# Shahriar1638/Hybrid-Language-Music-Clustering-VAE

Hardware: AMD Instinct MI355X
Metric: clips/sec mel+VAE train step, 128-mel x 128-frame, bs=256, 1/2/4/8 MI355X (higher is better)
Workload: dtype bf16; 1 GPU; Convolutional_VAE audio-only (BASELINE config[1]): PCM[256,65024] -> HIP mel-dB 128x128 -> z-score -> VAE fwd+bwd+Adam; per_gpu_batch=256, global_batch=256, mel=128x128, params=13304961, parallelism=dp1, world_size=1, launch=single process, pcm_batches=5 distinct batches in rotation (333 MB), execution=eager launches

## Files before the change

hybrid-language-music-clustering-vae_amd/csrc/gemm.hpp:

```cpp
#pragma once
#include "common.hpp"

namespace hlmc {

constexpr int kKCH = 8;
template <typename T>
constexpr int gemm_bk() { return kKCH * Vec16<T>::N; }

__device__ __forceinline__ int xcd_logical_block(int lin, int total) {
    const int xcd = lin & 7, idx = lin >> 3;
    const int q = total >> 3, r = total & 7;
    return (xcd < r ? xcd * (q + 1) : r * (q + 1) + (xcd - r) * q) + idx;
}

static __device__ __attribute__((aligned(16))) uint4 g_zero16 = {0u, 0u, 0u, 0u};
template <typename T> __device__ __attribute__((aligned(16))) uint4 g_one16 = {sizeof(T) == 2 ? 0x3F80u : 0x3F800000u, 0u, 0u, 0u};


template <typename T>
struct DenseLoader {
    const T* p;
    int ld, M, Kd;
    bool vec;
    struct Row {
// ... 29 lines not shown
    int Hi, Wi, C, Ho, Wo, M;
    int cshift;
    FastDiv dWo, dHo;
    struct Row {
        int64_t base;
        int flags;
    };
    struct Ctx {
        int64_t off;
        int reject;
    };
    __device__ void set_phase(int) {}
    __device__ int K() const { return 9 * C; }
    __device__ Row prep(int m) const {
        if (m >= M) return Row{0, 1 | 8};
        const int t = (int)dWo.div((uint32_t)m), ow = m - t * Wo;
        const int b = (int)dHo.div((uint32_t)t), oh = t - b * Ho;
        return Row{(((int64_t)b * Hi + 2 * oh - 1) * Wi + 2 * ow - 1) * C, 8 | (oh == 0 ? 2 : 0) | (ow == 0 ? 4 : 0)};
    }
    __device__ Ctx ctx(int k) const {
        const int tap = cshift >= 0 ? (k >> cshift) : k / C;
        const int ci = k - tap * C;
        const int kh = tap / 3, kw = tap - kh * 3;
        return Ctx{((int64_t)kh * Wi + kw) * C + ci, 1 | (kh == 0 ? 2 : 0) | (kw == 0 ? 4 : 0) | (tap >= 9 ? 8 : 0)};
    }
    __host__ __device__ bool vec_ok() const { return true; }
    __device__ uint4 load(const Row& rw, const Ctx& cx) const { return *reinterpret_cast<const uint4*>(addr(rw, cx)); }
    __device__ const void* addr(const Row& rw, const Ctx& cx) const {
        if (rw.flags & cx.reject) return &g_zero16;
        return x + rw.base + cx.off;
    }
};

__device__ __forceinline__ int sp_ntaps(int par) { return par ? 2 : 1; }
__device__ __forceinline__ int sp_kidx(int par, int t) { return par ? (t ? 2 : 0) : 1; }
__device__ __forceinline__ int sp_delta(int par, int t) { return (par && t == 0) ? 1 : 0; }

template <typename T>
struct SubpixelLoader {
    const T* x;
    int Hi, Wi, C, M;
    int cshift;
    int py, px, ntx, Kd;
    FastDiv dWi, dHi;
    struct Row {
        int64_t base;
        int flags;
    };
    struct Ctx {
        int64_t off;
        int reject;
    };
    __device__ void set_phase(int p) {
        py = p >> 1; px = p & 1;
        ntx = sp_ntaps(px);
        Kd = sp_ntaps(py) * ntx * C;
    }
    __device__ int K() const { return Kd; }
    __device__ Row prep(int m) const {
        if (m >= M) return Row{0, 1 | 8};
        const int t = (int)dWi.div((uint32_t)m), c = m - t * Wi;
        const int b = (int)dHi.div((uint32_t)t), r = t - b * Hi;
        return Row{(((int64_t)b * Hi + r) * Wi + c) * C, 8 | (r == Hi - 1 ? 2 : 0) | (c == Wi - 1 ? 4 : 0)};
    }
    __device__ Ctx ctx(int k) const {
        const int tt = cshift >= 0 ? (k >> cshift) : k / C;
        const int ci = k - tt * C;
        const int ty = ntx == 2 ? (tt >> 1) : tt, tx = ntx == 2 ? (tt & 1) : 0;
        const int dr = sp_delta(py, ty), dc = sp_delta(px, tx);
        return Ctx{((int64_t)dr * Wi + dc) * C + ci, 1 | (dr ? 2 : 0) | (dc ? 4 : 0) | (k >= Kd ? 8 : 0)};
    }
    __host__ __device__ bool vec_ok() const { return true; }
    __device__ uint4 load(const Row& rw, const Ctx& cx) const { return *reinterpret_cast<const uint4*>(addr(rw, cx)); }
    __device__ const void* addr(const Row& rw, const Ctx& cx) const {
        if (rw.flags & cx.reject) return &g_zero16;
        return x + rw.base + cx.off;
    }
};

template <typename T>
struct SubpixelWeight {
    const T* w;
    int C, N;
    int cshift;
    int py, px, ntx, Kd;
    struct Row {
        const T* r;
    };
    struct Ctx {
        int off;
    };
    __device__ void set_phase(int p) {
        py = p >> 1; px = p & 1;
        ntx = sp_ntaps(px);
        Kd = sp_ntaps(py) * ntx * C;
    }
    __device__ int K() const { return Kd; }
    __device__ Row prep(int n) const { return Row{n < N ? w + (int64_t)n * 9 * C : nullptr}; }
    __device__ Ctx ctx(int k) const {
        if (k >= Kd) return Ctx{-1};
        const int tt = cshift >= 0 ? (k >> cshift) : k / C;
        const int ci = k - tt * C;
        const int ty = ntx == 2 ? (tt >> 1) : tt, tx = ntx == 2 ? (tt & 1) : 0;
        return Ctx{(sp_kidx(py, ty) * 3 + sp_kidx(px, tx)) * C + ci};
    }
    __host__ __device__ bool vec_ok() const { return true; }
    __device__ uint4 load(const Row& rw, const Ctx& cx) const { return *reinterpret_cast<const uint4*>(addr(rw, cx)); }
    __device__ const void* addr(const Row& rw, const Ctx& cx) const {
        if (!rw.r || cx.off < 0) return &g_zero16;
        return rw.r + cx.off;
    }
};

template <typename OutT>
__device__ __forceinline__ void store4_round(OutT* p, float (&v)[4]) {
    if constexpr (sizeof(OutT) == 4) {
        *reinterpret_cast<float4*>(p) = make_float4(v[0], v[1], v[2], v[3]);
    } else {
        unsigned h[4];
#pragma unroll
        for (int k = 0; k < 4; ++k) {
            bf16 t = __float2bfloat16(v[k]);
            h[k] = *reinterpret_cast<unsigned short*>(&t);
            v[k] = __uint_as_float(h[k] << 16);
        }
        *reinterpret_cast<uint2*>(p) = make_uint2(h[0] | (h[1] << 16), h[2] | (h[3] << 16));
    }
}

template <typename OutT>
struct StoreRM {
    static constexpr int kStatMode = 0;
    static constexpr bool kDirectTn = true;
    OutT* out;
    const float* bias;
    int ld, act, accumulate;
    struct Row {
        OutT* r;
    };
    struct Quad {
        int64_t off;
    };
    __device__ void set_split(int) {}
    __device__ float colbias(int n) const { return bias ? bias[n] : 0.f; }
    __device__ Quad quad(int m) const { return Quad{(int64_t)m * ld}; }
    __device__ int64_t row_off(const Quad& q, int r) const { return q.off + (int64_t)r * ld; }
    __device__ float put(int64_t ro, int n, float v) const {
        if (act == 1) v = v > 0.f ? v : 0.f;
        OutT* o = out + ro + n;
        if (accumulate) v += to_f32<OutT>(*o);
        const OutT t = from_f32<OutT>(v);
        *o = t;
        return to_f32<OutT>(t);
    }
    __device__ void put4(int64_t ro, int n, float (&v)[4]) const {
        OutT* o = out + ro + n;
#pragma unroll
        for (int k = 0; k < 4; ++k) {
            if (act == 1) v[k] = v[k] > 0.f ? v[k] : 0.f;
            if (accumulate) v[k] += to_f32<OutT>(o[k]);
        }
        store4_round<OutT>(o, v);
    }
    __device__ float put_na(int64_t ro, int n, float v) const {
        if (act == 1) v = v > 0.f ? v : 0.f;
        const OutT t = from_f32<OutT>(v);
        out[ro + n] = t;
        return to_f32<OutT>(t);
    }
    __device__ float stored(int n, float v) const {
        if (bias) v += bias[n];
        if (act == 1) v = v > 0.f ? v : 0.f;
        return to_f32<OutT>(from_f32<OutT>(v));
    }
    __device__ void set_phase(int) {}
    __device__ Row row(int m) const { return Row{out + (int64_t)m * ld}; }
// ... 98 lines not shown
    }
    __device__ float stored(int n, float v) const {
        if (this->bias) v += this->bias[n];
        return to_f32<OutT>(from_f32<OutT>(v));
    }
    __device__ Row row(int m) const { return Row{m, fx.flat_row(m)}; }
    __device__ void store(const Row& rw, int n, float v) const {
        if (this->bias) v += this->bias[n];
        put_at(rw.m, rw.base, n, v);
    }
};

template <typename OutT>
struct StoreSubpixel {
    static constexpr int kStatMode = 0;
    OutT* out;
    const float* bias;
    int Hi, Wi, N;
    int py, px;
    FastDiv dWi, dHi;
    struct Row {
        OutT* r;
    };
    struct Quad {
        int64_t off;
        int m;
    };
    __device__ int64_t pix_off(int m) const {
        const int t = (int)dWi.div((uint32_t)m), c = m - t * Wi;
        const int b = (int)dHi.div((uint32_t)t), r = t - b * Hi;
        return (((int64_t)b * 2 * Hi + 2 * r + py) * (2 * Wi) + 2 * c + px) * N;
    }
    __device__ void set_split(int) {}
    __device__ float colbias(int n) const { return bias ? bias[n] : 0.f; }
    __device__ Quad quad(int m) const { return Quad{pix_off(m), m}; }
    __device__ int64_t row_off(const Quad& q, int r) const {
        return (Wi & 3) == 0 ? q.off + (int64_t)2 * r * N : pix_off(q.m + r);
    }
    __device__ float put(int64_t ro, int n, float v) const {
        const OutT t = from_f32<OutT>(v);
        out[ro + n] = t;
        return to_f32<OutT>(t);
    }
    __device__ void put4(int64_t ro, int n, float (&v)[4]) const { store4_round<OutT>(out + ro + n, v); }
    __device__ float put_na(int64_t ro, int n, float v) const { return put(ro, n, v); }
    __device__ float stored(int n, float v) const {
        if (bias) v += bias[n];
        return to_f32<OutT>(from_f32<OutT>(v));
    }
    __device__ void set_phase(int p) { py = p >> 1; px = p & 1; }
    __device__ Row row(int m) const {
        const int c = m % Wi, t = m / Wi;
        const int r = t % Hi, b = t / Hi;
        const int64_t pix = ((int64_t)b * 2 * Hi + 2 * r + py) * (2 * Wi) + 2 * c + px;
        return Row{out + pix * N};
    }
    __device__ void store(const Row& rw, int n, float v) const {
        if (bias) v += bias[n];
        rw.r[n] = from_f32<OutT>(v);
    }
};

template <class Base>
struct WithStats : Base {
    static constexpr int kStatMode = 1;
    XAcc acc;
};
template <class EP>
inline WithStats<EP> with_stats(const EP& ep, const XAcc& acc) {
    WithStats<EP> eps;
    static_cast<EP&>(eps) = ep;
    eps.acc = acc;
    return eps;
}

struct StorePartial {
    static constexpr int kStatMode = 0;
    float* ws;
    int M, N, S;
    int phase, split;
    struct Row {
        float* r;
    };
    __device__ void set_phase(int p) { phase = p; }
    __device__ Row row(int m) const { return Row{ws + (((int64_t)phase * S + split) * M + m) * N}; }
    __device__ void store(const Row& rw, int n, float v) const { rw.r[n] = v; }
    struct Quad {
        int64_t off;
    };
    __device__ void set_split(int z) { split = z; }
    __device__ float colbias(int) const { return 0.f; }
    __device__ Quad quad(int m) const { return Quad{(((int64_t)phase * S + split) * M + m) * N}; }
    __device__ int64_t row_off(const Quad& q, int r) const { return q.off + (int64_t)r * N; }
    __device__ float put(int64_t ro, int n, float v) const {
        ws[ro + n] = v;
        return v;
    }
    __device__ void put4(int64_t ro, int n, float (&v)[4]) const {
        *reinterpret_cast<float4*>(ws + ro + n) = make_float4(v[0], v[1], v[2], v[3]);
    }
};

template <int TM, int TN, class EP>
__device__ __forceinline__ void epilogue_tile(const EP& ep, const f32x4_t (&acc)[TM][TN], int mb, int nb, int lane,
                                              int M, int N, double (&cs)[TN], double (&cq)[TN]) {
    float bias[TN];
    int ncol[TN];
#pragma unroll
    for (int j = 0; j < TN; ++j) {
        ncol[j] = nb + j * 16 + (lane & 15);
        bias[j] = ncol[j] < N ? ep.colbias(ncol[j]) : 0.f;
        cs[j] = 0.0;
        cq[j] = 0.0;
    }
#pragma unroll
    for (int i = 0; i < TM; ++i) {
        const int m = mb + i * 16 + (lane >> 4) * 4;
        if (m >= M) continue;
        const typename EP::Quad q = ep.quad(m);
#pragma unroll
        for (int r = 0; r < 4; ++r) {
            if (m + r >= M) continue;
            const int64_t ro = ep.row_off(q, r);
#pragma unroll
            for (int j = 0; j < TN; ++j) {
// ... 74 lines not shown
                    sred[(wmi * 2 + 1) * BN + wn0 + j * 16 + 4 * (lane >> 4) + k] = cq[j * 4 + k];
                }
        }
    } else {
#pragma unroll
        for (int j = 0; j < TN; ++j) {
            double a = cs[j], q = cq[j];
            a += __shfl_xor(a, 16, 64);
            q += __shfl_xor(q, 16, 64);
            a += __shfl_xor(a, 32, 64);
            q += __shfl_xor(q, 32, 64);
            if (lane < 16) {
                sred[(wmi * 2 + 0) * BN + wn0 + j * 16 + lane] = a;
                sred[(wmi * 2 + 1) * BN + wn0 + j * 16 + lane] = q;
            }
        }
    }
}
template <bool TR>
__device__ __forceinline__ f32x4_t mfma_bf16(const bf16x8_t& a, const bf16x8_t& b, const f32x4_t& c) {
    if constexpr (TR) return __builtin_amdgcn_mfma_f32_16x16x32_bf16(b, a, c, 0, 0, 0);
    else return __builtin_amdgcn_mfma_f32_16x16x32_bf16(a, b, c, 0, 0, 0);
}
template <bool TR>
__device__ __forceinline__ f32x4_t mfma_f32(float a, float b, const f32x4_t& c) {
    if constexpr (TR) return __builtin_amdgcn_mfma_f32_16x16x4f32(b, a, c, 0, 0, 0);
    else return __builtin_amdgcn_mfma_f32_16x16x4f32(a, b, c, 0, 0, 0);
}

#define NT_BLOCK_COORDS()                                                                                  \
    const int gx_ = (int)gridDim.x, gy_ = (int)gridDim.y;                                                  \
    const int lin_ = (int)blockIdx.x + gx_ * ((int)blockIdx.y + gy_ * (int)blockIdx.z);                     \
    const int lg_ = remap ? xcd_logical_block(lin_, gx_ * gy_ * (int)gridDim.z) : 0;                       \
    const int phase = remap ? lg_ % gy_ : (int)blockIdx.y;                                                 \
    const int tile_ = remap ? (lg_ / gy_) % gx_ : (int)blockIdx.x;                                         \
    const int bz = remap ? lg_ / (gx_ * gy_) : (int)blockIdx.z;                                            \
    const int m0 = (tile_ / tiles_n) * BM, n0 = (tile_ % tiles_n) * BN;                                     \
    const int tile_m_ = tile_ / tiles_n

template <int KCH>
__device__ __forceinline__ int nt_lds_chunk(int row, int c) {
    if constexpr (KCH == 8) return c ^ (row & 7);
    else return c ^ ((0x78 >> (2 * ((row >> 2) & 3))) & 3);
}

template <typename T, int BM, int BN, int WM, int WN, int KCH, class AL, class BL, class EP, bool TR = false>
__global__ __launch_bounds__(256) void gemm_nt_kernel(AL al, BL bl, EP ep, int M, int N, int ksplit_len, int remap,
                                                      int ploop) {
    constexpr int V = Vec16<T>::N;
    constexpr int BK = KCH * V;
    constexpr int WAVES_N = BN / WN;
    static_assert((BM / WM) * WAVES_N == 4, "4 waves per block");
    constexpr int TM = WM / 16, TN = WN / 16;
    constexpr int ACH = BM * KCH, BCH = BN * KCH;
    constexpr int AR = (ACH + 255) / 256, BR = (BCH + 255) / 256;
    __shared__ __attribute__((aligned(16))) T As[2][BM * BK];
    __shared__ __attribute__((aligned(16))) T Bs[2][BN * BK];

    const int tid = threadIdx.x, lane = tid & 63, wave = tid >> 6;
    const int wm0 = (wave / WAVES_N) * WM, wn0 = (wave % WAVES_N) * WN;
    const int tiles_n = (N + BN - 1) / BN;
    NT_BLOCK_COORDS();
    typename AL::Row arow[AR];
    typename BL::Row brow[BR];
#pragma unroll
    for (int i = 0; i < AR; ++i) arow[i] = al.prep(m0 + ((tid + i * 256) / KCH));
#pragma unroll
    for (int i = 0; i < BR; ++i) brow[i] = bl.prep(n0 + ((tid + i * 256) / KCH));
    const int ph0 = ploop > 1 ? 0 : phase, ph1 = ploop > 1 ? ploop : phase + 1;
// ... 137 lines not shown
#pragma unroll
            for (int w = 0; w < WAVES_M; ++w) {
                a += sred[w][0][c];
                q += sred[w][1][c];
            }
            xacc_add_shard(ep.acc, shard, n, a);
            xacc_add_shard(ep.acc, shard, N + n, q);
        }
    }
    if (ph + 1 < ph1) __syncthreads();
    }
}

template <int N>
__device__ __forceinline__ void wait_vmcnt() {
    static_assert(N >= 0 && N < 64, "vmcnt range");
    asm volatile("s_waitcnt vmcnt(%0)" ::"n"(N) : "memory");
}
template <int GPW, int NS>
__device__ __forceinline__ void wait_stage(int ahead) {
    if constexpr (NS >= 4) {
        if (ahead >= 2) { wait_vmcnt<2 * GPW>(); return; }
    }
    if constexpr (NS >= 3) {
        if (ahead >= 1) { wait_vmcnt<GPW>(); return; }
    }
    wait_vmcnt<0>();
}
__device__ __forceinline__ void glds16(const void* g, void* l) {
    __builtin_amdgcn_global_load_lds((const __attribute__((address_space(1))) void*)g,
                                     (__attribute__((address_space(3))) void*)l, 16, 0, 0);
}

template <typename T, int BM, int BN, int WM, int WN, int NS, class AL, class BL, class EP, bool TR = false, int WPE = 1>
__global__ __launch_bounds__(256) __attribute__((amdgpu_waves_per_eu(WPE))) void gemm_nt_glds_kernel(
    AL al, BL bl, EP ep, int M, int N, int ksplit_len, int remap) {
    constexpr int V = Vec16<T>::N;
    constexpr int BK = 8 * V;
    constexpr int ASZ = BM * 128, BSZ = BN * 128, STG = ASZ + BSZ;
    constexpr int AI = BM / 8, BI = BN / 8;
    static_assert(AI % 4 == 0 && BI >= 4 && BI % 4 == 0, "tile rows per stage must split over 4 waves");
    constexpr int AIW = AI / 4, BIW = BI / 4, GPW = AIW + BIW;
    constexpr int WAVES_N = BN / WN;
    static_assert((BM / WM) * WAVES_N == 4, "4 waves per block");
    constexpr int TM = WM / 16, TN = WN / 16;
    __shared__ __attribute__((aligned(1024))) char smem[NS * STG];

    const int tid = threadIdx.x, lane = tid & 63, wave = tid >> 6;
    const int wm0 = (wave / WAVES_N) * WM, wn0 = (wave % WAVES_N) * WN;
    const int tiles_n = (N + BN - 1) / BN;
    NT_BLOCK_COORDS();
    al.set_phase(phase); bl.set_phase(phase); ep.set_phase(phase); ep.set_split(bz);
    const int K = al.K();
    const int kb = bz * ksplit_len;
    const int ke = min(K, kb + ksplit_len);
    const int nsteps = kb < ke ? (ke - kb + BK - 1) / BK : 0;

    f32x4_t acc[TM][TN];
#pragma unroll
    for (int i = 0; i < TM; ++i)
#pragma unroll
        for (int j = 0; j < TN; ++j) acc[i][j] = f32x4_t{0.f, 0.f, 0.f, 0.f};

    const int lrow = lane >> 3;
    const int lchunk = (lane & 7) ^ (lrow & 7);
    typename AL::Row arow[AIW];
    typename BL::Row brow[BIW];
#pragma unroll
    for (int i = 0; i < AIW; ++i) arow[i] = al.prep(m0 + (wave * AIW + i) * 8 + lrow);
#pragma unroll
    for (int i = 0; i < BIW; ++i) brow[i] = bl.prep(n0 + (wave * BIW + i) * 8 + lrow);
    auto issue = [&](int slot, int k0) {
        char* sb = smem + slot * STG;
        const int k = k0 + lchunk * V;
        const typename AL::Ctx ax = al.ctx(k);
        const typename BL::Ctx bx = bl.ctx(k);
#pragma unroll
        for (int i = 0; i < AIW; ++i) glds16(al.addr(arow[i], ax), sb + (wave * AIW + i) * 1024);
#pragma unroll
        for (int i = 0; i < BIW; ++i) glds16(bl.addr(brow[i], bx), sb + ASZ + (wave * BIW + i) * 1024);
    };

#pragma unroll
    for (int p = 0; p < NS - 1; ++p)
// ... 18 lines not shown
                for (int j = 0; j < TN; ++j) {
                    const int row = wn0 + j * 16 + (lane & 15);
                    bfr[j] = *reinterpret_cast<const bf16x8_t*>(sbb + row * 128 + ((c ^ (row & 7)) << 4));
                }
#pragma unroll
                for (int i = 0; i < TM; ++i)
#pragma unroll
                    for (int j = 0; j < TN; ++j)
                        acc[i][j] = mfma_bf16<TR>(af[i], bfr[j], acc[i][j]);
            }
        } else {
#pragma unroll
            for (int s = 0; s < BK / 4; ++s) {
                float af[TM], bfr[TN];
                const int q = lane >> 4;
#pragma unroll
                for (int i = 0; i < TM; ++i) {
                    const int row = wm0 + i * 16 + (lane & 15);
                    af[i] = *reinterpret_cast<const float*>(sa + row * 128 + ((s ^ (row & 7)) << 4) + q * 4);
                }
#pragma unroll
                for (int j = 0; j < TN; ++j) {
                    const int row = wn0 + j * 16 + (lane & 15);
                    bfr[j] = *reinterpret_cast<const float*>(sbb + row * 128 + ((s ^ (row & 7)) << 4) + q * 4);
                }
#pragma unroll
                for (int i = 0; i < TM; ++i)
#pragma unroll
                    for (int j = 0; j < TN; ++j)
                        acc[i][j] = mfma_f32<TR>(af[i], bfr[j], acc[i][j]);
            }
        }
    }
    double cs[TR ? TN * 4 : TN], cq[TR ? TN * 4 : TN];
    if constexpr (TR)
        epilogue_tile_t<TM, TN, EP, sizeof(T) == 2>(ep, acc, m0 + wm0, n0 + wn0, lane, M, N,
                                *reinterpret_cast<double(*)[TN][4]>(cs), *reinterpret_cast<double(*)[TN][4]>(cq));
    else
        epilogue_tile<TM, TN>(ep, acc, m0 + wm0, n0 + wn0, lane, M, N, cs, cq);
    if constexpr (EP::kStatMode != 0) {
        constexpr int WAVES_M = BM / WM;
        static_assert(WAVES_M * 2 * BN * 8 <= NS * STG, "stats scratch fits the staging ring");
        __syncthreads();
        double* sred = reinterpret_cast<double*>(smem);
        const int wmi = wave / WAVES_N;
        stats_to_lds<TR, TN, BN>(cs, cq, sred, wmi, wn0, lane);
        __syncthreads();
        const int shard = (int)((blockIdx.x + gridDim.x * blockIdx.y) % (unsigned)ep.acc.shards);
        for (int c = tid; c < BN; c += 256) {
            const int n = n0 + c;
            if (n >= N) continue;
            double a = 0.0, q = 0.0;
#pragma unroll
            for (int w = 0; w < WAVES_M; ++w) {
                a += sred[(w * 2 + 0) * BN + c];
                q += sred[(w * 2 + 1) * BN + c];
            }
            xacc_add_shard(ep.acc, shard, n, a);
            xacc_add_shard(ep.acc, shard, N + n, q);
        }
    }
}

struct StorePartialZ : StorePartial {
    __device__ void set_split(int z) { split = z; }
};

template <int VW>
using slab_t = std::conditional_t<VW == 4, float4, float>;
__device__ __forceinline__ void slab_add(float& a, float b) { a += b; }
__device__ __forceinline__ void slab_add(float4& a, const float4& b) { a.x += b.x; a.y += b.y; a.z += b.z; a.w += b.w; }
__device__ __forceinline__ float slab_at(float v, int) { return v; }
__device__ __forceinline__ float slab_at(const float4& v, int i) { return i == 0 ? v.x : i == 1 ? v.y : i == 2 ? v.z : v.w; }
template <int VW, int G, class I>
__device__ __forceinline__ slab_t<VW> slab_sum(const float* __restrict__ p, I st, int S, int g) {
    using V = slab_t<VW>;
    auto ld = [&](int k) { return *reinterpret_cast<const V*>(p + k * st); };
    V acc{};
    int k = g;
    for (; k + 3 * G < S; k += 4 * G) {
        const V a0 = ld(k), a1 = ld(k + G), a2 = ld(k + 2 * G), a3 = ld(k + 3 * G);
        slab_add(acc, a0); slab_add(acc, a1); slab_add(acc, a2); slab_add(acc, a3);
    }
    for (; k < S; k += G) slab_add(acc, ld(k));
    return acc;
}
template <class EP>
__device__ __forceinline__ void slab_store(const EP& ep, int ph, int m, int n, float v) {
    EP e = ep;
    e.set_phase(ph);
    e.store(e.row(m), n, v);
}
template <class EP>
__device__ __forceinline__ void slab_store(const EP& ep, int ph, int m, int n, const float4& v) {
    EP e = ep;
    e.set_phase(ph);
    const auto rw = e.row(m);
    e.store(rw, n, v.x);
    e.store(rw, n + 1, v.y);
    e.store(rw, n + 2, v.z);
    e.store(rw, n + 3, v.w);
}

template <int VW, class EP>
__global__ __launch_bounds__(256) void splitk_reduce_kernel(const float* __restrict__ ws, EP ep, int M, int N, int S,
                                                            int phases, FastDiv dN, FastDiv dM) {
    if constexpr (VW == 4) {
        const uint32_t e = (blockIdx.x * 256u + threadIdx.x) * 4u;
        if (e >= (uint32_t)phases * (uint32_t)M * (uint32_t)N) return;
        const uint32_t t = dN.div(e), n = e - t * (uint32_t)N;
        const uint32_t ph = dM.div(t), m = t - ph * (uint32_t)M;
        const uint32_t st = (uint32_t)M * (uint32_t)N;
        const float* p = ws + ((ph * (uint32_t)S) * (uint32_t)M + m) * (uint32_t)N + n;
        slab_store(ep, (int)ph, (int)m, (int)n, slab_sum<4, 1>(p, st, S, 0));
    } else {
        const int64_t total = (int64_t)phases * M * N, st = (int64_t)M * N;
        for (int64_t i = (int64_t)blockIdx.x * blockDim.x + threadIdx.x; i < total; i += (int64_t)gridDim.x * blockDim.x) {
            const int n = (int)(i % N);
            const int64_t t = i / N;
            const int m = (int)(t % M), ph = (int)(t / M);
            slab_store(ep, ph, m, n, slab_sum<1, 1>(ws + ((int64_t)ph * S * M + m) * N + n, st, S, 0));
        }
    }
}

template <class EP, int RU>
__global__ __launch_bounds__(256) void splitk_reduce_stats_kernel(const float* ws, EP ep, int M, int N, int S,
                                                                  int phases, XAcc acc) {
    __shared__ double red[2][256];
    const int tid = threadIdx.x, c = tid & 63, g = tid >> 6;
    const int ntc = N >> 6;
    const int tr = (int)(blockIdx.x / (unsigned)ntc);
    const int col = ((int)blockIdx.x - tr * ntc) * 64 + c;
    const int rows = phases * M;
    const unsigned st = (unsigned)M * (unsigned)N;
    const int r0 = tr * 4 * RU + g;
    unsigned off[RU];
    float s[RU];
#pragma unroll
    for (int u = 0; u < RU; ++u) {
        const int r = min(r0 + 4 * u, rows - 1);
        const int ph = r / M, m = r - ph * M;
        off[u] = ((unsigned)(ph * S) * (unsigned)M + (unsigned)m) * (unsigned)N + (unsigned)col;
        s[u] = 0.f;
    }
    int k = 0;
    for (; k + 2 <= S; k += 2) {
        float x0[RU], x1[RU];
#pragma unroll
        for (int u = 0; u < RU; ++u) {
            x0[u] = ws[off[u] + (unsigned)k * st];
            x1[u] = ws[off[u] + (unsigned)(k + 1) * st];
        }
#pragma unroll
        for (int u = 0; u < RU; ++u) {
            s[u] += x0[u];
            s[u] += x1[u];
        }
    }
    if (k < S)
#pragma unroll
        for (int u = 0; u < RU; ++u) s[u] += ws[off[u] + (unsigned)k * st];
    double a = 0.0, q = 0.0;
#pragma unroll
    for (int u = 0; u < RU; ++u) {
        const int r = r0 + 4 * u;
        if (r >= rows) break;
        const int ph = r / M, m = r - ph * M;
        EP e = ep;
        e.set_phase(ph);
        e.store(e.row(m), col, s[u]);
        const float v = e.stored(col, s[u]);
        a += v;
        q += (double)v * v;
    }
    red[0][tid] = a;
    red[1][tid] = q;
    __syncthreads();
    if (tid < 64) {
#pragma unroll
        for (int j = 1; j < 4; ++j) {
            a += red[0][j * 64 + tid];
            q += red[1][j * 64 + tid];
        }
        xacc_add(acc, col, a);
        xacc_add(acc, N + col, q);
    }
}

template <class L>
struct KRowStepped {
    struct Pre {
        typename L::Col cl;
        int j;
    };
// ... 414 lines not shown
```

hybrid-language-music-clustering-vae_amd/csrc/gemm_ops.hip:

```cpp
#include "gemm.hpp"
#include "halo.hpp"
#include "ops.hpp"

#include <algorithm>
#include <type_traits>
#include <cstdlib>

namespace hlmc {
namespace {

constexpr int kNtTargetBlocks = 512;
constexpr int kTnTargetBlocks = 192;
constexpr int kTnLongK = 131072;
constexpr int kTnKch8Min = 1024;
constexpr int kXcdRemapKinds = probe::kWgradS2 | probe::kLinearWgrad;

struct Plan {
    int S, ksl;
};
template <int BM_, int BN_, int WM_, int WN_>
struct Tile {
    static constexpr int BM = BM_, BN = BN_, WM = WM_, WN = WN_;
};
struct GemmPlan {
    int tiles;
    Plan pl;
    size_t slab_bytes;
};
inline Plan plan_nt(int tiles, int Kmax, int BK) {
    constexpr int target = kNtTargetBlocks;
    int S = 1;
    if (tiles < target / 2) {
        S = cdiv(target, tiles);
        S = std::min(S, std::max(1, Kmax / (2 * BK)));
    }
    int ksl = cdiv(cdiv(Kmax, S), BK) * BK;
    S = cdiv(Kmax, ksl);
    return {S, ksl};
}
inline Plan plan_tn(int tiles, int K, int BK) {
    const int target = K >= kTnLongK ? 2 * kTnTargetBlocks : kTnTargetBlocks;
    int S = cdiv(target, tiles);
    S = std::max(1, std::min(S, K / (4 * BK)));
    int ksl = cdiv(cdiv(K, S), BK) * BK;
    S = cdiv(K, ksl);
    return {S, ksl};
}

constexpr int kGldsSplitMax = 512;
inline int nt_pipe_select(int ksl, int S, int blocks) {
    if (S > 1 && blocks <= kGldsSplitMax) return 2;
    return ksl >= 1024 ? 2 : 0;
}

inline int xcd_remap_for_site() { return (kXcdRemapKinds & probe::g_site.kind) ? 1 : 0; }

constexpr int kPloopTiles = 1024;
inline bool use_ploop(int phases, int tmn, int pipe) { return phases >= 2 && pipe == 0 && tmn >= kPloopTiles; }

template <typename T, class TL, bool TR, class AL, class BL, class E>
void nt_kernel_launch_tr(hipStream_t s, dim3 grid, const AL& al, const BL& bl, const E& ep, int M, int N, int ksl,
                         bool long_k, int pipe) {
    constexpr int BM = TL::BM, BN = TL::BN, WM = TL::WM, WN = TL::WN;
    const int rm = xcd_remap_for_site();
    const int ploop = use_ploop((int)grid.y, (int)grid.x, pipe) ? (int)grid.y : 1;
    if (ploop > 1) grid.y = 1;
    HLMC_PROBE_BEGIN(s);
    if (pipe == 2)
        gemm_nt_glds_kernel<T, BM, BN, WM, WN, 2, AL, BL, E, TR, 2><<<grid, 256, 0, s>>>(al, bl, ep, M, N, ksl, rm);
    else if (long_k)
        gemm_nt_kernel<T, BM, BN, WM, WN, 8, AL, BL, E, TR><<<grid, 256, 0, s>>>(al, bl, ep, M, N, ksl, rm, ploop);
    else
        gemm_nt_kernel<T, BM, BN, WM, WN, 4, AL, BL, E, TR><<<grid, 256, 0, s>>>(al, bl, ep, M, N, ksl, rm, ploop);
    HLMC_PROBE_END(s);
}

template <typename T, class TL>
GemmPlan nt_plan(int M, int N, int Kmax, int phases) {
    const int tmn = cdiv(M, TL::BM) * cdiv(N, TL::BN);
    const Plan pl = plan_nt(tmn * phases, Kmax, gemm_bk<T>());
    return {tmn, pl, (size_t)phases * pl.S * M * N * sizeof(float)};
}
inline bool nt_long_k(int Kmax) { return Kmax >= 1024; }

template <typename T, class TL, bool TR, class AL, class BL>
int nt_partials(hipStream_t s, const AL& al, const BL& bl, const GemmPlan& gp, int M, int N, int Kmax, int phases, Ws ws,
                int pipe) {
    HLMC_CHECK_ARG(ws.p && ws.bytes >= gp.slab_bytes, "split-K workspace too small");
    StorePartialZ part;
    part.ws = ws.p; part.M = M; part.N = N; part.S = gp.pl.S; part.phase = 0; part.split = 0;
    nt_kernel_launch_tr<T, TL, TR>(s, dim3(gp.tiles, phases, gp.pl.S), al, bl, part, M, N, gp.pl.ksl, nt_long_k(Kmax),
                                   pipe);
    HLMC_LAUNCHED();
    return HLMC_OK;
}

template <typename T, class TL, bool TR, class AL, class BL, class EP>
int launch_nt(hipStream_t s, const AL& al, const BL& bl, const EP& ep, int M, int N, int Kmax, int phases, Ws ws,
              ops::ColStats* st = nullptr, bool dma_ok = true) {
    const GemmPlan gp = nt_plan<T, TL>(M, N, Kmax, phases);
    const int S = gp.pl.S, ksl = gp.pl.ksl;
    const int pipe = (dma_ok && TL::BN >= 32 && TL::BM >= 64) ? nt_pipe_select(ksl, S, gp.tiles * phases * S) : 0;
    const bool stats = st && st->acc.on();
    if (st) st->done = false;
    if (S == 1) {
        const dim3 grid(gp.tiles, phases, 1);
        const bool long_k = nt_long_k(Kmax);
        if (stats) nt_kernel_launch_tr<T, TL, TR>(s, grid, al, bl, with_stats(ep, st->acc), M, N, ksl, long_k, pipe);
        else nt_kernel_launch_tr<T, TL, TR>(s, grid, al, bl, ep, M, N, ksl, long_k, pipe);
        HLMC_LAUNCHED();
        if (stats) st->done = true;
        return HLMC_OK;
    }
    const int rc = nt_partials<T, TL, TR>(s, al, bl, gp, M, N, Kmax, phases, ws, pipe);
    if (rc != HLMC_OK) return rc;
    const bool idx32 = (double)phases * S * M * N < 2147483648.0;
    if (stats && N % 64 == 0 && idx32) {
        const int rows = phases * M, ntc = N / 64;
        const int RU = cdiv(rows, 128) * ntc >= 1024 ? 32 : cdiv(rows, 64) * ntc >= 1024 ? 16 : 8;
        const unsigned nb = (unsigned)(cdiv(rows, 4 * RU) * ntc);
        switch (RU) {
            case 32: splitk_reduce_stats_kernel<EP, 32><<<nb, 256, 0, s>>>(ws.p, ep, M, N, S, phases, st->acc); break;
            case 16: splitk_reduce_stats_kernel<EP, 16><<<nb, 256, 0, s>>>(ws.p, ep, M, N, S, phases, st->acc); break;
            default: splitk_reduce_stats_kernel<EP, 8><<<nb, 256, 0, s>>>(ws.p, ep, M, N, S, phases, st->acc); break;
        }
        HLMC_LAUNCHED();
        st->done = true;
        return HLMC_OK;
    }
    const int64_t total = (int64_t)phases * M * N;
    const FastDiv dN((uint32_t)N), dM((uint32_t)M);
    if (N % 4 == 0 && idx32 && ((uintptr_t)ws.p & 15) == 0) {
        const unsigned nb = (unsigned)((total / 4 + 255) / 256);
        splitk_reduce_kernel<4, EP><<<nb, 256, 0, s>>>(ws.p, ep, M, N, S, phases, dN, dM);
    } else {
        const int blocks = (int)std::min<int64_t>(4096, (total + 255) / 256);
        splitk_reduce_kernel<1, EP><<<blocks, 256, 0, s>>>(ws.p, ep, M, N, S, phases, dN, dM);
    }
    HLMC_LAUNCHED();
    return HLMC_OK;
}

template <class F>
auto with_nt_tile(int M, int N, int phases, F&& f) {
    const int t = cdiv(M, 128) * cdiv(N, 128) * phases;
    if (N >= 128 && !(t >= kNtTargetBlocks / 2 && t < kNtTargetBlocks)) return f(Tile<128, 128, 64, 64>{});
    if (N > 32) return f(Tile<128, 64, 32, 64>{});
    return f(Tile<128, 32, 32, 32>{});
}
template <typename T, class AL, class BL, class EP>
int dispatch_nt(hipStream_t s, const AL& al, const BL& bl, const EP& ep, int M, int N, int Kmax, int phases, Ws ws,
                ops::ColStats* st = nullptr) {
    return with_nt_tile(M, N, phases, [&](auto tl) {
        using TL = decltype(tl);
        if (N % 4 == 0) return launch_nt<T, TL, true>(s, al, bl, ep, M, N, Kmax, phases, ws, st);
        return launch_nt<T, TL, false>(s, al, bl, ep, M, N, Kmax, phases, ws, st);
    });
}
inline size_t split_ws(const GemmPlan& gp) { return gp.pl.S == 1 ? 0 : gp.slab_bytes; }
template <typename T>
size_t dispatch_nt_ws(int M, int N, int Kmax, int phases) {
    return with_nt_tile(M, N, phases, [&](auto tl) { return split_ws(nt_plan<T, decltype(tl)>(M, N, Kmax, phases)); });
}

template <class F>
auto with_linear_tile(int M, int N, F&& f) {
    if (M >= 1024 && N >= 128) return f(Tile<128, 128, 64, 64>{});
    return f(Tile<64, 64, 32, 32>{});
}
template <typename T, class AL, class BL, class EP>
// ... 55 lines not shown
}

template <class EP>
void reduce_splits(hipStream_t s, const float* ws, const EP& ep, int M, int N, int S) {
    if constexpr (std::is_same<EP, StoreWgradConv>::value) {
        if (S <= 4 && ep.C % 128 == 0 && (((uintptr_t)ws | (uintptr_t)ep.dW) & 15) == 0) {
            splitk_reduce_wgrad_conv_kernel<4><<<(unsigned)(M * (ep.C / 128)), 288, 0, s>>>(ws, ep, M, ep.C, S);
            return;
        }
        if (S <= 4 && ep.C % 32 == 0) {
            splitk_reduce_wgrad_conv_kernel<1><<<(unsigned)(M * (ep.C / 32)), 288, 0, s>>>(ws, ep, M, ep.C, S);
            return;
        }
    }
    const int64_t total = (int64_t)M * N;
    const bool v4 = N % 4 == 0 && ((uintptr_t)ws & 15) == 0;
    auto go = [&](auto gtag) {
        constexpr int G = decltype(gtag)::value;
        const int64_t per = v4 ? 4 * (256 / G) : 256 / G;
        const int64_t blocks = (total + per - 1) / per;
        if (v4) splitk_reduce_grouped_kernel<4, G, EP><<<(unsigned)blocks, 256, 0, s>>>(ws, ep, M, N, S);
        else splitk_reduce_grouped_kernel<1, G, EP><<<(unsigned)blocks, 256, 0, s>>>(ws, ep, M, N, S);
    };
    if (S >= 32) go(std::integral_constant<int, 8>{});
    else if (S >= 8) go(std::integral_constant<int, 4>{});
    else if (S >= 4) go(std::integral_constant<int, 2>{});
    else go(std::integral_constant<int, 1>{});
}

template <typename T, class TL>
GemmPlan tn_plan(int M, int N, int K) {
    const int tiles = cdiv(M, TL::BM) * cdiv(N, TL::BN);
    const Plan pl = plan_tn(tiles, K, gemm_bk<T>());
    return {tiles, pl, (size_t)pl.S * M * N * sizeof(float)};
}
template <typename T, class TL, class LL, class HL, class EP>
int launch_tn(hipStream_t s, const LL& ll, const HL& hl, const EP& ep, int M, int N, int K, Ws ws) {
    constexpr int BM = TL::BM, BN = TL::BN, WM = TL::WM, WN = TL::WN;
    const GemmPlan gp = tn_plan<T, TL>(M, N, K);
    const Plan pl = gp.pl;
    HLMC_CHECK_ARG(ws.p && ws.bytes >= gp.slab_bytes, "wgrad workspace too small");
    dim3 grid(gp.tiles, 1, pl.S);
    const int rm = xcd_remap_for_site();
    HLMC_PROBE_BEGIN(s);
    const bool vec = ll.vec_ok() && hl.vec_ok();
    constexpr int NTH = 64 * (BM / WM) * (BN / WN);
    auto go = [&](auto out) {
        using OUT = decltype(out);
        if (pl.ksl >= kTnKch8Min) {
            if (vec) gemm_tn_kernel<T, BM, BN, WM, WN, 8, LL, HL, true, OUT><<<grid, NTH, 0, s>>>(ll, hl, out, M, N, K, pl.ksl, rm);
            else gemm_tn_kernel<T, BM, BN, WM, WN, 8, LL, HL, false, OUT><<<grid, NTH, 0, s>>>(ll, hl, out, M, N, K, pl.ksl, rm);
        } else {
            if (vec) gemm_tn_kernel<T, BM, BN, WM, WN, 4, LL, HL, true, OUT><<<grid, NTH, 0, s>>>(ll, hl, out, M, N, K, pl.ksl, rm);
            else gemm_tn_kernel<T, BM, BN, WM, WN, 4, LL, HL, false, OUT><<<grid, NTH, 0, s>>>(ll, hl, out, M, N, K, pl.ksl, rm);
        }
    };
    if constexpr (tn_direct<EP>::value) {
        if (pl.S == 1) {
            go(TnDirect<EP>{ep});
            HLMC_PROBE_END(s);
            HLMC_LAUNCHED();
            return HLMC_OK;
        }
    }
    go(TnSlab{ws.p});
    HLMC_PROBE_END(s);
    HLMC_LAUNCHED();
// ... 284 lines not shown
size_t linear_wgrad_ws(int Mb, int N, int K) {
    return std::max(dispatch_tn_ws<T>(N, K, Mb), dispatch_tn_ws<T>(N, K + 1, Mb));
}

#define INST(T)                                                                                                     \
    template int conv_s2<T>(hipStream_t, const T*, int, int, int, int, const T*, const float*, int, T*, Ws,         \
                            ColStats*, const BnInput*, const FlatOut*);                                             \
    template bool conv_s2_takes_input_bn<T>(int, int, int, int, int);                                              \
    template bool subpixel_takes_input_bn<T>(int, int, int, int, int);                                             \
    template size_t conv_s2_ws<T>(int, int, int, int, int);                                                        \
    template int subpixel<T>(hipStream_t, const T*, int, int, int, int, const T*, const float*, int, T*, Ws,        \
                             ColStats*, const BnInput*);                                                                             \
    template size_t subpixel_ws<T>(int, int, int, int, int);                                                       \
    template int wgrad_s2<T>(hipStream_t, const T*, int, int, int, int, const T*, int, float*, Ws, XAcc, float*);  \
    template size_t wgrad_s2_ws<T>(int, int, int, int, int);                                                       \
    template int linear<T, T>(hipStream_t, const T*, int, int, int, const T*, int, const float*, int, T*, int, int, \
                              int, Ws, const T*, const NhwcOut*);                                                  \
    template size_t linear_ws<T>(int, int, int);                                                                   \
    template int linear_partials<T>(hipStream_t, const T*, int, int, int, const T*, int, int, Ws, int*);           \
    template size_t linear_partials_ws<T>(int, int, int);                                                          \
    template int linear_wgrad_pair<T>(hipStream_t, const T*, int, const T*, int, int, int, int, float*, float*,    \
                                      float*, float*, Ws);                                                         \
    template int linear_wgrad<T>(hipStream_t, const T*, int, const T*, int, int, int, int, float*, float*, Ws);    \
    template size_t linear_wgrad_ws<T>(int, int, int);

INST(float)
INST(bf16)
#undef INST
template int linear<bf16, float>(hipStream_t, const bf16*, int, int, int, const bf16*, int, const float*, int, float*,
                                 int, int, int, Ws, const float*, const NhwcOut*);

}
}
#ifdef HLMC_TN_TS
extern "C" int hlmc_debug_tn_ts(void* host, int nblocks) {
    return (int)hipMemcpyFromSymbol(host, HIP_SYMBOL(hlmc::g_tn_ts), (size_t)nblocks * 32, 0, hipMemcpyDeviceToHost);
}
#endif
```

Baseline: 144,100 clips/s.

## Size split-K slabs per subpixel phase to skip empty K-splits

For subpixel (transposed-conv) GEMMs with four phases, each phase has a different K (1, 2, 2 or 4 taps times C), yet every phase used to launch the same number of K-splits sized for Kmax. Now the plan computes per-phase split counts into a flat z-dimension of slab units, and blocks map their z index back to phase and split, so splits that would cover only zero-padded K are no longer launched, stored or reduced. The reduce kernels take per-phase slab offsets and counts, and the workspace shrinks to match. A compile-time gated timestamp probe is also added but is off by default.

```diff
diff --git a/hybrid-language-music-clustering-vae_amd/csrc/gemm.hpp b/hybrid-language-music-clustering-vae_amd/csrc/gemm.hpp
--- a/hybrid-language-music-clustering-vae_amd/csrc/gemm.hpp
+++ b/hybrid-language-music-clustering-vae_amd/csrc/gemm.hpp
@@ -85,7 +85,8 @@
     }
 };
 
-__device__ __forceinline__ int sp_ntaps(int par) { return par ? 2 : 1; }
+__host__ __device__ __forceinline__ int sp_ntaps(int par) { return par ? 2 : 1; }
+__host__ __device__ __forceinline__ int sp_phase_taps(int p) { return sp_ntaps(p >> 1) * sp_ntaps(p & 1); }
 __device__ __forceinline__ int sp_kidx(int par, int t) { return par ? (t ? 2 : 0) : 1; }
 __device__ __forceinline__ int sp_delta(int par, int t) { return (par && t == 0) ? 1 : 0; }
 
@@ -107,7 +108,7 @@
     __device__ void set_phase(int p) {
         py = p >> 1; px = p & 1;
         ntx = sp_ntaps(px);
-        Kd = sp_ntaps(py) * ntx * C;
+        Kd = sp_phase_taps(p) * C;
     }
     __device__ int K() const { return Kd; }
     __device__ Row prep(int m) const {
@@ -146,7 +147,7 @@
     __device__ void set_phase(int p) {
         py = p >> 1; px = p & 1;
         ntx = sp_ntaps(px);
-        Kd = sp_ntaps(py) * ntx * C;
+        Kd = sp_phase_taps(p) * C;
     }
     __device__ int K() const { return Kd; }
     __device__ Row prep(int n) const { return Row{n < N ? w + (int64_t)n * 9 * C : nullptr}; }
@@ -195,6 +196,7 @@
         int64_t off;
     };
     __device__ void set_split(int) {}
+    __device__ void unit(int&, int&) const {}
     __device__ float colbias(int n) const { return bias ? bias[n] : 0.f; }
     __device__ Quad quad(int m) const { return Quad{(int64_t)m * ld}; }
     __device__ int64_t row_off(const Quad& q, int r) const { return q.off + (int64_t)r * ld; }
@@ -359,6 +361,7 @@
         return (((int64_t)b * 2 * Hi + 2 * r + py) * (2 * Wi) + 2 * c + px) * N;
     }
     __device__ void set_split(int) {}
+    __device__ void unit(int&, int&) const {}
     __device__ float colbias(int n) const { return bias ? bias[n] : 0.f; }
     __device__ Quad quad(int m) const { return Quad{pix_off(m), m}; }
     __device__ int64_t row_off(const Quad& q, int r) const {
@@ -401,23 +404,39 @@
     return eps;
 }
 
+struct SlabUnits {
+    int first[5];
+    __host__ __device__ int at(int p) const {
+        return p <= 0 ? first[0] : p == 1 ? first[1] : p == 2 ? first[2] : p == 3 ? first[3] : first[4];
+    }
+    __host__ __device__ int count(int p) const { return at(p + 1) - at(p); }
+};
+
 struct StorePartial {
     static constexpr int kStatMode = 0;
     float* ws;
-    int M, N, S;
+    int M, N;
+    SlabUnits un;
+    int flat;
     int phase, split;
     struct Row {
         float* r;
     };
+    __device__ int64_t slab() const { return un.at(phase) + split; }
     __device__ void set_phase(int p) { phase = p; }
-    __device__ Row row(int m) const { return Row{ws + (((int64_t)phase * S + split) * M + m) * N}; }
+    __device__ Row row(int m) const { return Row{ws + (slab() * M + m) * N}; }
     __device__ void store(const Row& rw, int n, float v) const { rw.r[n] = v; }
     struct Quad {
         int64_t off;
     };
     __device__ void set_split(int z) { split = z; }
+    __device__ void unit(int& ph, int& z) const {
+        if (!flat) return;
+        ph = (z >= un.first[1]) + (z >= un.first[2]) + (z >= un.first[3]);
+        z -= un.at(ph);
+    }
     __device__ float colbias(int) const { return 0.f; }
-    __device__ Quad quad(int m) const { return Quad{(((int64_t)phase * S + split) * M + m) * N}; }
+    __device__ Quad quad(int m) const { return Quad{(slab() * M + m) * N}; }
     __device__ int64_t row_off(const Quad& q, int r) const { return q.off + (int64_t)r * N; }
     __device__ float put(int64_t ro, int n, float v) const {
         ws[ro + n] = v;
@@ -558,9 +577,10 @@
     const int gx_ = (int)gridDim.x, gy_ = (int)gridDim.y;                                                  \
     const int lin_ = (int)blockIdx.x + gx_ * ((int)blockIdx.y + gy_ * (int)blockIdx.z);                     \
     const int lg_ = remap ? xcd_logical_block(lin_, gx_ * gy_ * (int)gridDim.z) : 0;                       \
-    const int phase = remap ? lg_ % gy_ : (int)blockIdx.y;                                                 \
+    int phase = remap ? lg_ % gy_ : (int)blockIdx.y;                                                       \
     const int tile_ = remap ? (lg_ / gy_) % gx_ : (int)blockIdx.x;                                         \
-    const int bz = remap ? lg_ / (gx_ * gy_) : (int)blockIdx.z;                                            \
+    int bz = remap ? lg_ / (gx_ * gy_) : (int)blockIdx.z;                                                  \
+    ep.unit(phase, bz);                                                                                    \
     const int m0 = (tile_ / tiles_n) * BM, n0 = (tile_ % tiles_n) * BN;                                     \
     const int tile_m_ = tile_ / tiles_n
 
@@ -764,6 +784,28 @@
                                      (__attribute__((address_space(3))) void*)l, 16, 0, 0);
 }
 
+#ifdef HLMC_NT_TS
+__device__ unsigned long long g_nt_ts[8192][5];
+__device__ int g_nt_pair;
+#define NT_TS_PAIR() if (g_nt_pair && gridDim.y == 4) phase = (0x87 >> (2 * phase)) & 3
+#define NT_TS(i) const unsigned long long nt_ts##i##_ = wall_clock64()
+#define NT_TS_END()                                                                                                \
+    do {                                                                                                           \
+        __syncthreads();                                                                                           \
+        if (threadIdx.x == 0 && (unsigned)lin_ < 8192u) {                                                          \
+            unsigned long long* o_ = g_nt_ts[lin_];                                                                \
+            o_[0] = nt_ts0_; o_[1] = nt_ts1_; o_[2] = wall_clock64();                                              \
+            o_[3] = (unsigned long long)phase | (unsigned long long)nsteps << 8 | (unsigned long long)bz << 24;    \
+            o_[4] = (unsigned long long)__builtin_amdgcn_s_getreg(4 | 31 << 11) |                                  \
+                    (unsigned long long)__builtin_amdgcn_s_getreg(20 | 31 << 11) << 32;                            \
+        }                                                                                                          \
+    } while (0)
+#else
+#define NT_TS(i)
+#define NT_TS_PAIR()
+#define NT_TS_END()
+#endif
+
 template <typename T, int BM, int BN, int WM, int WN, int NS, class AL, class BL, class EP, bool TR = false, int WPE = 1>
 __global__ __launch_bounds__(256) __attribute__((amdgpu_waves_per_eu(WPE))) void gemm_nt_glds_kernel(
     AL al, BL bl, EP ep, int M, int N, int ksplit_len, int remap) {
@@ -781,7 +823,9 @@
     const int tid = threadIdx.x, lane = tid & 63, wave = tid >> 6;
     const int wm0 = (wave / WAVES_N) * WM, wn0 = (wave % WAVES_N) * WN;
     const int tiles_n = (N + BN - 1) / BN;
+    NT_TS(0);
     NT_BLOCK_COORDS();
+    NT_TS_PAIR();
     al.set_phase(phase); bl.set_phase(phase); ep.set_phase(phase); ep.set_split(bz);
     const int K = al.K();
     const int kb = bz * ksplit_len;
@@ -866,6 +910,7 @@
             }
         }
     }
+    NT_TS(1);
     double cs[TR ? TN * 4 : TN], cq[TR ? TN * 4 : TN];
     if constexpr (TR)
         epilogue_tile_t<TM, TN, EP, sizeof(T) == 2>(ep, acc, m0 + wm0, n0 + wn0, lane, M, N,
@@ -894,6 +939,7 @@
             xacc_add_shard(ep.acc, shard, N + n, q);
         }
     }
+    NT_TS_END();
 }
 
 struct StorePartialZ : StorePartial {
@@ -937,29 +983,29 @@
 }
 
 template <int VW, class EP>
-__global__ __launch_bounds__(256) void splitk_reduce_kernel(const float* __restrict__ ws, EP ep, int M, int N, int S,
-                                                            int phases, FastDiv dN, FastDiv dM) {
+__global__ __launch_bounds__(256) void splitk_reduce_kernel(const float* __restrict__ ws, EP ep, int M, int N,
+                                                            SlabUnits un, int phases, FastDiv dN, FastDiv dM) {
     if constexpr (VW == 4) {
         const uint32_t e = (blockIdx.x * 256u + threadIdx.x) * 4u;
         if (e >= (uint32_t)phases * (uint32_t)M * (uint32_t)N) return;
         const uint32_t t = dN.div(e), n = e - t * (uint32_t)N;
         const uint32_t ph = dM.div(t), m = t - ph * (uint32_t)M;
         const uint32_t st = (uint32_t)M * (uint32_t)N;
-        const float* p = ws + ((ph * (uint32_t)S) * (uint32_t)M + m) * (uint32_t)N + n;
-        slab_store(ep, (int)ph, (int)m, (int)n, slab_sum<4, 1>(p, st, S, 0));
+        const float* p = ws + ((uint32_t)un.at((int)ph) * (uint32_t)M + m) * (uint32_t)N + n;
+        slab_store(ep, (int)ph, (int)m, (int)n, slab_sum<4, 1>(p, st, un.count((int)ph), 0));
     } else {
         const int64_t total = (int64_t)phases * M * N, st = (int64_t)M * N;
         for (int64_t i = (int64_t)blockIdx.x * blockDim.x + threadIdx.x; i < total; i += (int64_t)gridDim.x * blockDim.x) {
             const int n = (int)(i % N);
             const int64_t t = i / N;
             const int m = (int)(t % M), ph = (int)(t / M);
-            slab_store(ep, ph, m, n, slab_sum<1, 1>(ws + ((int64_t)ph * S * M + m) * N + n, st, S, 0));
+            slab_store(ep, ph, m, n, slab_sum<1, 1>(ws + ((int64_t)un.at(ph) * M + m) * N + n, st, un.count(ph), 0));
         }
     }
 }
 
 template <class EP, int RU>
-__global__ __launch_bounds__(256) void splitk_reduce_stats_kernel(const float* ws, EP ep, int M, int N, int S,
+__global__ __launch_bounds__(256) void splitk_reduce_stats_kernel(const float* ws, EP ep, int M, int N, SlabUnits un,
                                                                   int phases, XAcc acc) {
     __shared__ double red[2][256];
     const int tid = threadIdx.x, c = tid & 63, g = tid >> 6;
@@ -970,31 +1016,36 @@
     const unsigned st = (unsigned)M * (unsigned)N;
     const int r0 = tr * 4 * RU + g;
     unsigned off[RU];
+    int cnt[RU];
     float s[RU];
+    int S = 0;
 #pragma unroll
     for (int u = 0; u < RU; ++u) {
         const int r = min(r0 + 4 * u, rows - 1);
         const int ph = r / M, m = r - ph * M;
-        off[u] = ((unsigned)(ph * S) * (unsigned)M + (unsigned)m) * (unsigned)N + (unsigned)col;
+        off[u] = ((unsigned)un.at(ph) * (unsigned)M + (unsigned)m) * (unsigned)N + (unsigned)col;
+        cnt[u] = un.count(ph);
+        S = max(S, cnt[u]);
         s[u] = 0.f;
     }
+    auto ld = [&](int u, int k) { return ws[off[u] + (unsigned)min(k, cnt[u] - 1) * st]; };
     int k = 0;
     for (; k + 2 <= S; k += 2) {
         float x0[RU], x1[RU];
 #pragma unroll
         for (int u = 0; u < RU; ++u) {
-            x0[u] = ws[off[u] + (unsigned)k * st];
-            x1[u] = ws[off[u] + (unsigned)(k + 1) * st];
+            x0[u] = ld(u, k);
+            x1[u] = ld(u, k + 1);
         }
 #pragma unroll
         for (int u = 0; u < RU; ++u) {
-            s[u] += x0[u];
-            s[u] += x1[u];
+            s[u] += k < cnt[u] ? x0[u] : 0.f;
+            s[u] += k + 1 < cnt[u] ? x1[u] : 0.f;
         }
     }
     if (k < S)
 #pragma unroll
-        for (int u = 0; u < RU; ++u) s[u] += ws[off[u] + (unsigned)k * st];
+        for (int u = 0; u < RU; ++u) s[u] += k < cnt[u] ? ld(u, k) : 0.f;
     double a = 0.0, q = 0.0;
 #pragma unroll
     for (int u = 0; u < RU; ++u) {
diff --git a/hybrid-language-music-clustering-vae_amd/csrc/gemm_ops.hip b/hybrid-language-music-clustering-vae_amd/csrc/gemm_ops.hip
--- a/hybrid-language-music-clustering-vae_amd/csrc/gemm_ops.hip
+++ b/hybrid-language-music-clustering-vae_amd/csrc/gemm_ops.hip
@@ -25,6 +25,7 @@
 struct GemmPlan {
     int tiles;
     Plan pl;
+    SlabUnits un;
     size_t slab_bytes;
 };
 inline Plan plan_nt(int tiles, int Kmax, int BK) {
@@ -75,11 +76,15 @@
     HLMC_PROBE_END(s);
 }
 
+inline int nt_phase_k(int phases, int p, int Kmax) { return phases == 1 ? Kmax : sp_phase_taps(p) * (Kmax / 4); }
 template <typename T, class TL>
 GemmPlan nt_plan(int M, int N, int Kmax, int phases) {
     const int tmn = cdiv(M, TL::BM) * cdiv(N, TL::BN);
     const Plan pl = plan_nt(tmn * phases, Kmax, gemm_bk<T>());
-    return {tmn, pl, (size_t)phases * pl.S * M * N * sizeof(float)};
+    SlabUnits un{};
+    for (int p = 0; p < 4; ++p)
+        un.first[p + 1] = un.first[p] + (p < phases ? cdiv(nt_phase_k(phases, p, Kmax), pl.ksl) : 0);
+    return {tmn, pl, un, (size_t)un.first[4] * M * N * sizeof(float)};
 }
 inline bool nt_long_k(int Kmax) { return Kmax >= 1024; }
 
@@ -88,9 +93,9 @@
                 int pipe) {
     HLMC_CHECK_ARG(ws.p && ws.bytes >= gp.slab_bytes, "split-K workspace too small");
     StorePartialZ part;
-    part.ws = ws.p; part.M = M; part.N = N; part.S = gp.pl.S; part.phase = 0; part.split = 0;
-    nt_kernel_launch_tr<T, TL, TR>(s, dim3(gp.tiles, phases, gp.pl.S), al, bl, part, M, N, gp.pl.ksl, nt_long_k(Kmax),
-                                   pipe);
+    part.ws = ws.p; part.M = M; part.N = N; part.un = gp.un; part.flat = phases > 1; part.phase = 0; part.split = 0;
+    nt_kernel_launch_tr<T, TL, TR>(s, dim3(gp.tiles, 1, gp.un.first[4]), al, bl, part, M, N, gp.pl.ksl,
+                                   nt_long_k(Kmax), pipe);
     HLMC_LAUNCHED();
     return HLMC_OK;
 }
@@ -114,15 +119,15 @@
     }
     const int rc = nt_partials<T, TL, TR>(s, al, bl, gp, M, N, Kmax, phases, ws, pipe);
     if (rc != HLMC_OK) return rc;
-    const bool idx32 = (double)phases * S * M * N < 2147483648.0;
+    const bool idx32 = (double)gp.un.first[4] * M * N < 2147483648.0;
     if (stats && N % 64 == 0 && idx32) {
         const int rows = phases * M, ntc = N / 64;
         const int RU = cdiv(rows, 128) * ntc >= 1024 ? 32 : cdiv(rows, 64) * ntc >= 1024 ? 16 : 8;
         const unsigned nb = (unsigned)(cdiv(rows, 4 * RU) * ntc);
         switch (RU) {
-            case 32: splitk_reduce_stats_kernel<EP, 32><<<nb, 256, 0, s>>>(ws.p, ep, M, N, S, phases, st->acc); break;
-            case 16: splitk_reduce_stats_kernel<EP, 16><<<nb, 256, 0, s>>>(ws.p, ep, M, N, S, phases, st->acc); break;
-            default: splitk_reduce_stats_kernel<EP, 8><<<nb, 256, 0, s>>>(ws.p, ep, M, N, S, phases, st->acc); break;
+            case 32: splitk_reduce_stats_kernel<EP, 32><<<nb, 256, 0, s>>>(ws.p, ep, M, N, gp.un, phases, st->acc); break;
+            case 16: splitk_reduce_stats_kernel<EP, 16><<<nb, 256, 0, s>>>(ws.p, ep, M, N, gp.un, phases, st->acc); break;
+            default: splitk_reduce_stats_kernel<EP, 8><<<nb, 256, 0, s>>>(ws.p, ep, M, N, gp.un, phases, st->acc); break;
         }
         HLMC_LAUNCHED();
         st->done = true;
@@ -132,10 +137,10 @@
     const FastDiv dN((uint32_t)N), dM((uint32_t)M);
     if (N % 4 == 0 && idx32 && ((uintptr_t)ws.p & 15) == 0) {
         const unsigned nb = (unsigned)((total / 4 + 255) / 256);
-        splitk_reduce_kernel<4, EP><<<nb, 256, 0, s>>>(ws.p, ep, M, N, S, phases, dN, dM);
+        splitk_reduce_kernel<4, EP><<<nb, 256, 0, s>>>(ws.p, ep, M, N, gp.un, phases, dN, dM);
     } else {
         const int blocks = (int)std::min<int64_t>(4096, (total + 255) / 256);
-        splitk_reduce_kernel<1, EP><<<blocks, 256, 0, s>>>(ws.p, ep, M, N, S, phases, dN, dM);
+        splitk_reduce_kernel<1, EP><<<blocks, 256, 0, s>>>(ws.p, ep, M, N, gp.un, phases, dN, dM);
     }
     HLMC_LAUNCHED();
     return HLMC_OK;
@@ -257,7 +262,7 @@
 GemmPlan tn_plan(int M, int N, int K) {
     const int tiles = cdiv(M, TL::BM) * cdiv(N, TL::BN);
     const Plan pl = plan_tn(tiles, K, gemm_bk<T>());
-    return {tiles, pl, (size_t)pl.S * M * N * sizeof(float)};
+    return {tiles, pl, SlabUnits{{0, pl.S, pl.S, pl.S, pl.S}}, (size_t)pl.S * M * N * sizeof(float)};
 }
 template <typename T, class TL, class LL, class HL, class EP>
 int launch_tn(hipStream_t s, const LL& ll, const HL& hl, const EP& ep, int M, int N, int K, Ws ws) {
@@ -608,6 +613,14 @@
 
 }
 }
+#ifdef HLMC_NT_TS
+extern "C" int hlmc_debug_nt_ts(void* host, int nblocks) {
+    return (int)hipMemcpyFromSymbol(host, HIP_SYMBOL(hlmc::g_nt_ts), (size_t)nblocks * 40, 0, hipMemcpyDeviceToHost);
+}
+extern "C" int hlmc_debug_nt_pair(int on) {
+    return (int)hipMemcpyToSymbol(HIP_SYMBOL(hlmc::g_nt_pair), &on, sizeof(int), 0, hipMemcpyHostToDevice);
+}
+#endif
 #ifdef HLMC_TN_TS
 extern "C" int hlmc_debug_tn_ts(void* host, int nblocks) {
     return (int)hipMemcpyFromSymbol(host, HIP_SYMBOL(hlmc::g_tn_ts), (size_t)nblocks * 32, 0, hipMemcpyDeviceToHost);
```

New measurement: 143,800 clips/s. About the same (-0.2%).
